# mravanelli/pytorch-kaldi

Hardware: AMD Instinct MI355X
Metric: train_frames_per_sec (higher is better)
Workload: dtype bf16

## Files before the change

include/pk_amd.h:

```cpp
#ifndef PK_AMD_H
#define PK_AMD_H

#include <stdint.h>

#ifdef __cplusplus
extern "C" {
#endif

#define PK_PREC_F32 0
#define PK_PREC_BF16 1

#define PK_ACT_LINEAR 0
#define PK_ACT_RELU 1
#define PK_ACT_TANH 2
#define PK_ACT_SIGMOID 3
#define PK_ACT_LEAKY_RELU 4
#define PK_ACT_ELU 5

#define PK_CELL_LIGRU 0
#define PK_CELL_RNN 1
#define PK_CELL_LSTM 2
#define PK_CELL_GRU 3
#define PK_CELL_MINGRU 4

#define PK_REC_STEPWISE 0
#define PK_REC_PERSISTENT 1

int pk_version(void);
const char* pk_last_error(void);
int pk_num_cu(void);

int pk_gemm(void* stream, int prec, int M, int N, int K, float alpha, const float* A, int64_t a_rs,
            int64_t a_cs, const float* B, int64_t b_rs, int64_t b_cs, float beta, float* C, int64_t ldc,
            const float* bias, int splitk, float* workspace);
void pk_gemm_f32_set_form(int form);

int pk_gemm_bf16_tile_m(int M);
int pk_gemm_bf16_auto_splitk(int M, int N, int K);
int pk_gemm_bf16_auto_splitk_cus(int M, int N, int K, int cus);
void pk_gemm_bf16_set_tile(int tile);
int pk_gemm_bf16(void* stream, int M, int N, int K, float alpha, const uint16_t* A, int64_t lda, int a_kc,
                 const uint16_t* B, int64_t ldb, int b_kc, float beta, float* C, int64_t ldc, const float* bias,
                 int splitk, float* workspace);
int64_t pk_gemm_bf16_stats_floats(int M, int N);
int pk_gemm_bf16_stats(void* stream, int M, int N, int K, float alpha, const uint16_t* A, int64_t lda, int a_kc,
                       const uint16_t* B, int64_t ldb, int b_kc, float* C, int64_t ldc, const float* bias, float* stats,
                       int* row_blocks);
int pk_cvt_bf16(void* stream, const float* src, int64_t ld_src, int64_t rows, int nseg, int seglen, int segpad,
                uint16_t* dst, int64_t ld_dst);

int64_t pk_bn_partial_floats(int64_t M, int64_t N);
int pk_bn_stats(void* stream, const float* x, int64_t ldx, int64_t M, int64_t N, float* partial, float* mean,
                float* var);
int pk_bn_stats_merge(void* stream, const float* partial, int rb, int64_t N, float* mean, float* var);
int pk_bn_finalize(void* stream, int64_t N, const float* mean, const float* var, const float* gamma,
                   const float* beta, float eps, float* scale, float* shift, float* running_mean,
                   float* running_var, float momentum, double count);
int pk_bn_finalize_gates(void* stream, int G, int H, const float* mean, const float* var, const float* gamma,
                         const float* beta, float eps, float* scale, float* shift, float* const* running_mean,
                         float* const* running_var, int64_t* const* num_batches, float momentum, double count);
int pk_bn_stats_merge_finalize_gates(void* stream, const float* partial, int rb, int G, int H, float* mean, float* var,
                                     const float* gamma, const float* beta, float eps, float* scale, float* shift,
                                     float* const* running_mean, float* const* running_var, int64_t* const* num_batches,
                                     float momentum, double count);
int pk_affine_act_fwd(void* stream, const float* x, int64_t ldx, int64_t M, int64_t N, const float* scale,
                      const float* shift, int act, const float* mask, float* y, int64_t ldy);
int pk_act_bwd(void* stream, const float* dy, const float* a, const float* mask, int act, int64_t n, float* g);
int pk_bn_bwd_reduce(void* stream, const float* g, const float* g2, int64_t ldg, const float* x, int64_t ldx,
                     int64_t M, int64_t N, const float* mean, const float* var, float eps, float* partial,
                     float* sum_g, float* sum_gx);
int pk_bn_bwd_apply(void* stream, const float* g, const float* g2, int64_t ldg, const float* x, int64_t ldx,
                    int64_t M, int64_t N, const float* mean, const float* var, float eps, const float* gamma,
                    const float* sum_g, const float* sum_gx, double count, float* dx, int64_t lddx);
int pk_bn_bwd_bf16(void* stream, const uint16_t* g0, const uint16_t* g1, int64_t g_pitch, int G, int H, const float* x,
                   int64_t ldx, int64_t M, const float* mean, const float* var, float eps, const float* gamma,
                   double count, float* partial, float* sum_g, float* sum_gx, uint16_t* out, int64_t out_pitch,
                   float* acc_beta, float* acc_gamma);
int pk_bn_act_bwd_small_covers(int64_t M, int64_t N);
int pk_bn_act_bwd_small(void* stream, const float* dy, const float* a, const float* mask, int act, const float* z,
                        const float* mean, const float* var, float eps, const float* gamma, int64_t M, int64_t N,
                        uint16_t* dzb, int64_t ldb, float* dz, float* sum_g, float* sum_gx, float* acc_beta,
                        float* acc_gamma, float* db, float* acc_bias);
int pk_colsum(void* stream, const float* g, const float* g2, int64_t ldg, int64_t M, int64_t N, float* partial,
              float* out);
int pk_add(void* stream, const float* a, const float* b, int64_t n, float* out);

int pk_mt19937_bernoulli(void* stream, uint32_t* state, int64_t n, float keep, float* out);

int pk_sinc_bank_fwd(void* stream, const float* low_hz, const float* band_hz, const float* n_, const float* window, int N, int K,
                     float sample_rate, float min_low, float min_band, float* filt, float* mx, int32_t* kstar);
int pk_sinc_bank_bwd(void* stream, const float* g, const float* low_hz, const float* band_hz, const float* n_, const float* window,
                     const float* mx, const int32_t* kstar, int N, int K, float sample_rate, float min_low, float min_band,
                     float* dlow, float* dband);
// ... 150 lines not shown
```

pytorch-kaldi_amd/_lib.py:

```python
import ctypes
import os
import re
import threading

HERE = os.path.dirname(os.path.abspath(__file__))
LIB_PATH = os.path.join(HERE, "lib", "libpk_amd.so")
HEADER = os.path.join(HERE, "..", "include", "pk_amd.h")

_lock = threading.Lock()
_lib = None

c_void_p, c_int, c_float, c_double, c_int64 = ctypes.c_void_p, ctypes.c_int, ctypes.c_float, ctypes.c_double, ctypes.c_int64
P = c_void_p

SIGNATURES = {
    "pk_version": (c_int, []),
    "pk_last_error": (ctypes.c_char_p, []),
    "pk_num_cu": (c_int, []),
    "pk_gemm": (c_int, [P, c_int, c_int, c_int, c_int, c_float, P, c_int64, c_int64, P, c_int64, c_int64, c_float, P,
                        c_int64, P, c_int, P]),
    "pk_gemm_f32_set_form": (None, [c_int]),
    "pk_gemm_bf16_tile_m": (c_int, [c_int]),
    "pk_gemm_bf16_auto_splitk": (c_int, [c_int, c_int, c_int]),
    "pk_gemm_bf16_set_tile": (None, [c_int]),
    "pk_gemm_bf16": (c_int, [P, c_int, c_int, c_int, c_float, P, c_int64, c_int, P, c_int64, c_int, c_float, P, c_int64, P,
                             c_int, P]),
    "pk_gemm_bf16_stats_floats": (c_int64, [c_int, c_int]),
    "pk_gemm_bf16_stats": (c_int, [P, c_int, c_int, c_int, c_float, P, c_int64, c_int, P, c_int64, c_int, P, c_int64, P, P, P]),
    "pk_bn_stats_merge": (c_int, [P, P, c_int, c_int64, P, P]),
    "pk_cvt_bf16": (c_int, [P, P, c_int64, c_int64, c_int, c_int, c_int, P, c_int64]),
    "pk_bn_partial_floats": (c_int64, [c_int64, c_int64]),
    "pk_bn_stats": (c_int, [P, P, c_int64, c_int64, c_int64, P, P, P]),
    "pk_bn_finalize": (c_int, [P, c_int64, P, P, P, P, c_float, P, P, P, P, c_float, c_double]),
    "pk_bn_finalize_gates": (c_int, [P, c_int, c_int, P, P, P, P, c_float, P, P, P, P, P, c_float, c_double]),
    "pk_bn_stats_merge_finalize_gates": (c_int, [P, P, c_int, c_int, c_int, P, P, P, P, c_float, P, P, P, P, P, c_float,
                                                 c_double]),
    "pk_affine_act_fwd": (c_int, [P, P, c_int64, c_int64, c_int64, P, P, c_int, P, P, c_int64]),
    "pk_act_bwd": (c_int, [P, P, P, P, c_int, c_int64, P]),
    "pk_bn_bwd_reduce": (c_int, [P, P, P, c_int64, P, c_int64, c_int64, c_int64, P, P, c_float, P, P, P]),
    "pk_bn_bwd_apply": (c_int, [P, P, P, c_int64, P, c_int64, c_int64, c_int64, P, P, c_float, P, P, P, c_double, P,
                                c_int64]),
    "pk_bn_bwd_bf16": (c_int, [P, P, P, c_int64, c_int, c_int, P, c_int64, c_int64, P, P, c_float, P, c_double, P, P, P, P,
                               c_int64, P, P]),
    "pk_colsum": (c_int, [P, P, P, c_int64, c_int64, c_int64, P, P]),
    "pk_add": (c_int, [P, P, P, c_int64, P]),
    "pk_mt19937_bernoulli": (c_int, [P, P, c_int64, c_float, P]),
    "pk_sinc_bank_fwd": (c_int, [P, P, P, P, P, c_int, c_int, c_float, c_float, c_float, P, P, P]),
    "pk_sinc_bank_bwd": (c_int, [P, P, P, P, P, P, P, P, c_int, c_int, c_float, c_float, c_float, P, P]),
    "pk_ln_last_act_drop_fwd": (c_int, [P, P, c_int64, c_int, c_int, P, P, c_float, c_int, P, P, P, P, P]),
    "pk_ln_last_act_drop_bwd": (c_int, [P, P, P, P, P, c_int64, c_int, c_int, P, P, P, c_float, c_int, P, P]),
    "pk_layernorm_fwd": (c_int, [P, P, c_int64, c_int64, P, P, c_float, P, P, P]),
    "pk_layernorm_bwd": (c_int, [P, P, P, c_int64, c_int64, P, P, P, c_float, P, P]),
    "pk_logsoftmax_fwd": (c_int, [P, P, c_int64, c_int64, P]),
    "pk_logsoftmax_bwd": (c_int, [P, P, P, c_int64, c_int64, P]),
    "pk_logsoftmax_bwd_ld": (c_int, [P, P, P, c_int64, c_int64, P, c_int64]),
    "pk_logsoftmax_fwd_ld": (c_int, [P, P, c_int64, c_int64, c_int64, P]),
    "pk_logsoftmax_fwd_ld_argmax": (c_int, [P, P, c_int64, c_int64, c_int64, P, P]),
    "pk_logsoftmax_bwd_bf16_partial_floats": (c_int64, [c_int64, c_int64]),
    "pk_logsoftmax_bwd_bf16": (c_int, [P, P, P, c_int64, c_int64, P, c_int64, P, P]),
    "pk_nll_err_partial_floats": (c_int64, [c_int64]),
    "pk_nll_err_fwd": (c_int, [P, P, P, c_int64, c_int64, c_int64, P, P, P, P]),
    "pk_nll_err_fwd_argmax": (c_int, [P, P, P, P, c_int64, c_int64, c_int64, P, P, P, P]),
    "pk_nll_logsoftmax_bwd_bf16": (c_int, [P, P, P, P, P, c_int64, c_int64, c_int64, P, c_int64, P, P]),
    "pk_logsoftmax_bwd_bf16_p": (c_int, [P, P, P, c_int64, c_int64, P, c_int64, c_int64, P, P]),
    "pk_nll_logsoftmax_bwd_bf16_p": (c_int, [P, P, P, P, P, c_int64, c_int64, c_int64, P, c_int64, c_int64, P, P]),
    "pk_rec_num_saved": (c_int, [c_int]),
    "pk_rec_num_gates": (c_int, [c_int]),
    "pk_conv1d_pool_dgrad": (c_int, [P, P, P, P, c_int, c_int, c_int, c_int, c_int, c_int, P, P]),
    "pk_conv_bf16_covers": (c_int, [c_int, c_int, c_int, c_int]),
    "pk_conv_bf16_work_floats": (c_int64, [c_int, c_int, c_int, c_int, c_int, c_int, c_int]),
    "pk_conv1d_pool_fwd_bf16": (c_int, [P, P, P, P, c_int, c_int, c_int, c_int, c_int, c_int, P, P, P]),
    "pk_conv1d_pool_bwd_bf16": (c_int, [P, P, P, P, P, c_int, c_int, c_int, c_int, c_int, c_int, P, P, P]),
    "pk_bn_act_bwd_small_covers": (c_int, [c_int64, c_int64]),
    "pk_bn_act_bwd_small": (c_int, [P, P, P, P, c_int, P, P, P, c_float, P, c_int64, c_int64, P, c_int64, P, P, P, P, P, P, P]),
    "pk_rec_work_floats": (c_int64, [c_int, c_int, c_int, c_int, c_int]),
    "pk_rec_ln_saved_floats": (c_int64, [c_int, c_int, c_int, c_int]),
    "pk_rec_ln_work_floats": (c_int64, [c_int, c_int, c_int, c_int]),
# ... 268 lines not shown
```

pytorch-kaldi_amd/csrc/pk_gemm_bf16.hip:

```cpp
#include <stdlib.h>

#include "pk_common.h"

namespace {

constexpr int TM = 128, TN = 128, TK = 64;
typedef short s4v __attribute__((ext_vector_type(4)));

struct BArgs {
    int M, N, K;
    float alpha, beta;
    const unsigned short* A;
    long lda;
    const unsigned short* B;
    long ldb;
    float* C;
    long ldc;
    const float* bias;
    float* ws;
    int k_per_split;
    int tiles_m, tiles_n;
    int items, per_xcd;
    const unsigned short* zeros;
    float* stats;
// ... 669 lines not shown
                bf16x8 a[2], b[2];
#pragma unroll
                for (int i = 0; i < 2; ++i) a[i] = frag_km32(cur + wm * 4096, i * 16, kk, lane);
#pragma unroll
                for (int j = 0; j < 2; ++j) b[j] = frag_km32(cur + 8192 + wn * 4096, j * 16, kk, lane);
#pragma unroll
                for (int i = 0; i < 2; ++i)
#pragma unroll
                    for (int j = 0; j < 2; ++j)
                        acc[i][j] = __builtin_amdgcn_mfma_f32_16x16x32_bf16(b[j], a[i], acc[i][j], 0, 0, 0);
            }
        }
        __syncthreads();
    }
    const bool vec_ok = (p.ldc & 3) == 0 && (((uintptr_t)p.C) & 15) == 0;
#pragma unroll
    for (int i = 0; i < 2; ++i) {
        const int row = m0 + wm * 32 + i * 16 + (lane & 15);
        if (row >= p.M) continue;
#pragma unroll
        for (int j = 0; j < 2; ++j) {
            const int col = n0 + wn * 32 + j * 16 + (lane >> 4) * 4;
            float* dst = p.C + (long)row * p.ldc + col;
            if (vec_ok && col + 3 < p.N) {
                f32x4 o;
#pragma unroll
                for (int r = 0; r < 4; ++r) o[r] = p.alpha * acc[i][j][r] + (p.bias ? p.bias[col + r] : 0.f);
                if (p.beta != 0.f) {
                    const f32x4 c = *reinterpret_cast<const f32x4*>(dst);
#pragma unroll
                    for (int r = 0; r < 4; ++r) o[r] += p.beta * c[r];
                }
                *reinterpret_cast<f32x4*>(dst) = o;
            } else {
#pragma unroll
                for (int r = 0; r < 4; ++r) {
                    if (col + r >= p.N) continue;
                    float o = p.alpha * acc[i][j][r] + (p.bias ? p.bias[col + r] : 0.f);
                    if (p.beta != 0.f) o += p.beta * dst[r];
                    dst[r] = o;
                }
            }
        }
    }
}

constexpr int PIECE = 16384;
template <int V>
struct BoolK {
    static constexpr int value = V;
};

typedef unsigned int u32x2v __attribute__((ext_vector_type(2)));
template <bool KC>
__device__ __forceinline__ bf16x8 frag8(const unsigned char* buf, int sub, int kk, int lane) {
    if (KC) {
        return frag<true>(buf, sub, kk, lane);
    } else {
        const int g = lane >> 4, i = lane & 15;
        const int col = sub + (i & 3) * 4;
        u32x2v h[2];
#pragma unroll
        for (int hh = 0; hh < 2; ++hh) {
            const int kr = kk * 32 + g * 8 + hh * 4 + (i >> 2);
            const int ps = (col >> 3) ^ swz_km(kr);
            const unsigned addr = (unsigned)(size_t)(const __attribute__((address_space(3))) unsigned char*)(buf + kr * 256 + ps * 16 + (col & 7) * 2);
            asm volatile("ds_read_b64_tr_b16 %0, %1" : "=v"(h[hh]) : "v"(addr) : "memory");
        }
        typedef unsigned int u32x4v __attribute__((ext_vector_type(4)));
        const u32x4v o = u32x4v{h[0][0], h[0][1], h[1][0], h[1][1]};
        return __builtin_bit_cast(bf16x8, o);
    }
}
template <bool ANY_ASM>
__device__ __forceinline__ void frag_wait() {
    if (ANY_ASM) {
        asm volatile("s_waitcnt lgkmcnt(0)" ::: "memory");
        __builtin_amdgcn_sched_barrier(0);
    }
}

template <bool KC>
struct PieceSrc {
    TileSrc<KC, 512> t;
    const unsigned short* base;
    long ld;
    int r0, rmax;
    __device__ __forceinline__ void init(const unsigned short* b, long l, int r0_, int rmax_, int k0, int tid) {
        base = b; ld = l; r0 = r0_; rmax = rmax_;
        t.init(b, l, r0_, rmax_, k0, tid);
    }
    template <bool CHECKED>
    __device__ __forceinline__ void issue(int k0, int kend, const unsigned short* zeros, unsigned char* slot, int tid, int wave) {
        if (!CHECKED || k0 + TK <= kend) {
            t.issue(slot, wave);
        } else {
            stage<KC, 512>(base, ld, r0, rmax, k0, kend, zeros, slot, tid, wave);
#pragma unroll
            for (int j = 0; j < 2; ++j) t.a[j] += t.step;
        }
    }
};

__device__ __forceinline__ void store_frag(const BArgs& p, const f32x4 v, int row, int col, int split, bool vec_ok) {
    if (row >= p.M || col >= p.N) return;
    float* dst = p.ws ? p.ws + ((long)split * p.M + row) * p.N + col : p.C + (long)row * p.ldc + col;
    if (vec_ok && col + 3 < p.N) {
        f32x4 o = v;
        if (p.ws == nullptr) {
#pragma unroll
            for (int r = 0; r < 4; ++r) o[r] = p.alpha * v[r] + (p.bias ? p.bias[col + r] : 0.f);
            if (p.beta != 0.f) {
                const f32x4 c = *reinterpret_cast<const f32x4*>(dst);
#pragma unroll
                for (int r = 0; r < 4; ++r) o[r] += p.beta * c[r];
            }
        }
        *reinterpret_cast<f32x4*>(dst) = o;
    } else {
#pragma unroll
        for (int r = 0; r < 4; ++r) {
            if (col + r >= p.N) continue;
            float o = v[r];
            if (p.ws == nullptr) {
                o = p.alpha * o + (p.bias ? p.bias[col + r] : 0.f);
                if (p.beta != 0.f) o += p.beta * dst[r];
            }
            dst[r] = o;
        }
    }
}

__device__ __forceinline__ void tile_colstats(const BArgs& p, const f32x4 (&acc)[2][2][4][2], int m0, int n0, int tm, int wm,
                                              int wn, int lane, float* sh) {
    const int nrows = (p.M - m0) < 256 ? (p.M - m0) : 256;
    __syncthreads();
    float part[2][2][4];
#pragma unroll
    for (int pass = 0; pass < 2; ++pass) {
        float mu[2][2][4];
        if (pass == 1) {
#pragma unroll
            for (int bh = 0; bh < 2; ++bh)
#pragma unroll
                for (int j = 0; j < 2; ++j)
#pragma unroll
                    for (int r = 0; r < 4; ++r) {
                        const int cl = bh * 128 + wn * 32 + j * 16 + (lane >> 4) * 4 + r;
                        mu[bh][j][r] = (sh[cl] + sh[256 + cl]) / (float)nrows;
                    }
        }
#pragma unroll
        for (int bh = 0; bh < 2; ++bh)
#pragma unroll
            for (int j = 0; j < 2; ++j)
#pragma unroll
                for (int r = 0; r < 4; ++r) {
                    float t = 0.f;
#pragma unroll
                    for (int ah = 0; ah < 2; ++ah)
#pragma unroll
                        for (int i = 0; i < 4; ++i) {
                            const bool in = ah * 128 + wm * 64 + i * 16 + (lane & 15) < nrows;
                            const float v = acc[ah][bh][i][j][r];
                            const float d = pass == 0 ? v : v - mu[bh][j][r];
                            t += in ? (pass == 0 ? d : d * d) : 0.f;
                        }
#pragma unroll
                    for (int off = 1; off < 16; off <<= 1) t += __shfl_xor(t, off);
                    part[bh][j][r] = t;
                }
        if ((lane & 15) == 0) {
#pragma unroll
            for (int bh = 0; bh < 2; ++bh)
#pragma unroll
                for (int j = 0; j < 2; ++j)
#pragma unroll
                    for (int r = 0; r < 4; ++r)
                        sh[pass * 512 + wm * 256 + bh * 128 + wn * 32 + j * 16 + (lane >> 4) * 4 + r] = part[bh][j][r];
        }
        __syncthreads();
    }
    const int c = threadIdx.x;
    if (c < 256 && n0 + c < p.N) {
        const float mean_v = (sh[c] + sh[256 + c]) / (float)nrows;
        const float m2_v = sh[512 + c] + sh[768 + c];
        float* o = p.stats + ((long)tm * p.N + n0 + c) * 3;
        o[0] = (float)nrows;
        o[1] = p.alpha * mean_v + (p.bias ? p.bias[n0 + c] : 0.f);
        o[2] = p.alpha * p.alpha * m2_v;
    }
}

#define PK_VMCNT(n) asm volatile("s_waitcnt vmcnt(" #n ")" ::: "memory")

template <bool A_KC, bool B_KC>
__global__ __launch_bounds__(512, 1) void gemm_bf16_256_kernel(BArgs p) {
    extern __shared__ __attribute__((aligned(1024))) unsigned char smem[];
    const int tid = threadIdx.x, lane = tid & 63, wave = tid >> 6;
    const int wm = wave >> 2, wn = wave & 3;
    const int item = (blockIdx.x & 7) * p.per_xcd + (blockIdx.x >> 3);
    if (item >= p.items) return;
    const int tn = item % p.tiles_n;
    const int tm = (item / p.tiles_n) % p.tiles_m;
    const int split = item / (p.tiles_n * p.tiles_m);
    const int m0 = tm * 256, n0 = tn * 256;
    const int kbeg = split * p.k_per_split;
    const int kend = min(p.K, kbeg + p.k_per_split);
    const int nk = (kend - kbeg + TK - 1) / TK;
    const bool a1_live = m0 + 128 < p.M, b1_live = n0 + 128 < p.N;

    f32x4 acc[2][2][4][2];
#pragma unroll
    for (int a = 0; a < 2; ++a)
#pragma unroll
        for (int b = 0; b < 2; ++b)
#pragma unroll
            for (int i = 0; i < 4; ++i)
#pragma unroll
                for (int j = 0; j < 2; ++j) acc[a][b][i][j] = f32x4{0.f, 0.f, 0.f, 0.f};

    PieceSrc<A_KC> sa0, sa1;
    PieceSrc<B_KC> sb0, sb1;
    sa0.init(p.A, p.lda, m0, p.M, kbeg, tid);
    sa1.init(p.A, p.lda, m0 + 128, p.M, kbeg, tid);
    sb0.init(p.B, p.ldb, n0, p.N, kbeg, tid);
    sb1.init(p.B, p.ldb, n0 + 128, p.N, kbeg, tid);
    auto slot = [&](int kt, int piece) { return smem + (((kt & 1) * 4 + piece) * PIECE); };
    auto issueA0 = [&](int kt, auto C) { sa0.template issue<decltype(C)::value != 0>(kbeg + kt * TK, kend, p.zeros, slot(kt, 0), tid, wave); };
    auto issueB0 = [&](int kt, auto C) { sb0.template issue<decltype(C)::value != 0>(kbeg + kt * TK, kend, p.zeros, slot(kt, 1), tid, wave); };
    auto issueB1 = [&](int kt, auto C) { sb1.template issue<decltype(C)::value != 0>(kbeg + kt * TK, kend, p.zeros, slot(kt, 2), tid, wave); };
    auto issueA1 = [&](int kt, auto C) { sa1.template issue<decltype(C)::value != 0>(kbeg + kt * TK, kend, p.zeros, slot(kt, 3), tid, wave); };

    issueA0(0, BoolK<1>()); issueB0(0, BoolK<1>()); issueB1(0, BoolK<1>()); issueA1(0, BoolK<1>());
    issueA0(1, BoolK<1>()); issueB0(1, BoolK<1>()); issueB1(1, BoolK<1>());
    PK_VMCNT(10);
    __builtin_amdgcn_s_barrier();
    if (wm == 1) __builtin_amdgcn_s_barrier();

    bf16x8 a[4][2], b[2][2][2];
#define PK_MFMA_BLOCK(AH, BH)                                                                                         \
    do {                                                                                                              \
// ... 9 lines not shown
        __builtin_amdgcn_sched_barrier(0);                 \
        __builtin_amdgcn_s_barrier();                      \
    } while (0)
    auto ktile = [&](int kt, auto FQC, auto CKC) {
        constexpr bool FQ = decltype(FQC)::value != 0;
        issueA1(kt + 1, CKC);
#pragma unroll
        for (int kk = 0; kk < 2; ++kk) {
#pragma unroll
            for (int j = 0; j < 2; ++j) b[0][j][kk] = frag8<B_KC>(slot(kt, 1), wn * 32 + j * 16, kk, lane);
#pragma unroll
            for (int i = 0; i < 4; ++i) a[i][kk] = frag8<A_KC>(slot(kt, 0), wm * 64 + i * 16, kk, lane);
        }
        PK_VMCNT(10);
        PK_END_L();
        PK_MFMA_BLOCK(0, 0);
        __builtin_amdgcn_s_barrier();
        issueA0(kt + 2, CKC);
#pragma unroll
        for (int kk = 0; kk < 2; ++kk)
#pragma unroll
            for (int j = 0; j < 2; ++j) b[1][j][kk] = frag8<B_KC>(slot(kt, 2), wn * 32 + j * 16, kk, lane);
        PK_VMCNT(10);
        PK_END_L();
        if (FQ || b1_live) PK_MFMA_BLOCK(0, 1);
        __builtin_amdgcn_s_barrier();
        issueB0(kt + 2, CKC);
#pragma unroll
        for (int kk = 0; kk < 2; ++kk)
#pragma unroll
            for (int i = 0; i < 4; ++i) a[i][kk] = frag8<A_KC>(slot(kt, 3), wm * 64 + i * 16, kk, lane);
        PK_END_L();
        if (FQ || (a1_live && b1_live)) PK_MFMA_BLOCK(1, 1);
        __builtin_amdgcn_s_barrier();
        issueB1(kt + 2, CKC);
        PK_VMCNT(10);
        __builtin_amdgcn_s_barrier();
        if (FQ || a1_live) PK_MFMA_BLOCK(1, 0);
        __builtin_amdgcn_s_barrier();
    };
    const int nk_full = (kend - kbeg) / TK;
    auto run = [&](auto FQC) {
        int kt = 0;
        for (; kt + 2 < nk_full; ++kt) ktile(kt, FQC, BoolK<0>());
        for (; kt < nk; ++kt) ktile(kt, FQC, BoolK<1>());
    };
    if (a1_live && b1_live) run(BoolK<1>());
    else run(BoolK<0>());
#undef PK_MFMA_BLOCK
#undef PK_END_L
    if (wm == 0) __builtin_amdgcn_s_barrier();
    PK_VMCNT(0);
    if constexpr (A_KC && B_KC) {
        if (p.stats != nullptr) tile_colstats(p, acc, m0, n0, tm, wm, wn, lane, reinterpret_cast<float*>(smem));
    }
    const bool vec_ok = (((uintptr_t)(p.ws ? p.ws : p.C) & 15) == 0) && (((p.ws ? (long)p.N : p.ldc) & 3) == 0);
    const bool interior = m0 + 256 <= p.M && n0 + 256 <= p.N;
    if (vec_ok && interior && (p.ws != nullptr || p.beta == 0.f)) {
        const bool direct = p.ws == nullptr;
        float* base = direct ? p.C : p.ws + (long)split * p.M * p.N;
        const long ld = direct ? p.ldc : (long)p.N;
        const float alpha = direct ? p.alpha : 1.f;
#pragma unroll
        for (int bh = 0; bh < 2; ++bh)
#pragma unroll
            for (int j = 0; j < 2; ++j) {
                const int col = n0 + bh * 128 + wn * 32 + j * 16 + (lane >> 4) * 4;
                f32x4 bv = f32x4{0.f, 0.f, 0.f, 0.f};
                if (direct && p.bias != nullptr) {
#pragma unroll
                    for (int r = 0; r < 4; ++r) bv[r] = p.bias[col + r];
                }
#pragma unroll
                for (int ah = 0; ah < 2; ++ah)
#pragma unroll
                    for (int i = 0; i < 4; ++i) {
                        const int row = m0 + ah * 128 + wm * 64 + i * 16 + (lane & 15);
                        const f32x4 v = acc[ah][bh][i][j];
                        f32x4 o;
#pragma unroll
                        for (int r = 0; r < 4; ++r) o[r] = alpha * v[r] + bv[r];
                        *reinterpret_cast<f32x4*>(base + (long)row * ld + col) = o;
                    }
            }
        return;
    }
#pragma unroll
    for (int ah = 0; ah < 2; ++ah)
#pragma unroll
        for (int bh = 0; bh < 2; ++bh)
#pragma unroll
            for (int i = 0; i < 4; ++i)
#pragma unroll
                for (int j = 0; j < 2; ++j)
                    store_frag(p, acc[ah][bh][i][j], m0 + ah * 128 + wm * 64 + i * 16 + (lane & 15),
                               n0 + bh * 128 + wn * 32 + j * 16 + (lane >> 4) * 4, split, vec_ok);
}

__global__ void splitk_reduce_bf_kernel(const float* __restrict__ ws, int splitk, int M, int N, float alpha, float beta,
                                        const float* __restrict__ bias, float* __restrict__ C, long ldc) {
    const long total = (long)M * N;
    if ((N & 3) == 0 && (ldc & 3) == 0 && (((uintptr_t)C | (uintptr_t)ws) & 15) == 0) {
        const long quads = total >> 2;
        for (long qd = blockIdx.x * (long)blockDim.x + threadIdx.x; qd < quads; qd += (long)gridDim.x * blockDim.x) {
            const long i = qd << 2;
            const int row = (int)(i / N), col = (int)(i - (long)row * N);
            f32x4 s = f32x4{0.f, 0.f, 0.f, 0.f};
            for (int k0 = 0; k0 < splitk; k0 += 8) {
                f32x4 t[8];
#pragma unroll
                for (int j = 0; j < 8; ++j) t[j] = *reinterpret_cast<const f32x4*>(ws + (long)(k0 + j < splitk ? k0 + j : splitk - 1) * total + i);
#pragma unroll
                for (int j = 0; j < 8; ++j)
#pragma unroll
                    for (int e = 0; e < 4; ++e) s[e] += (k0 + j < splitk) ? t[j][e] : 0.f;
            }
            float* c = C + (long)row * ldc + col;
            f32x4 o;
#pragma unroll
            for (int e = 0; e < 4; ++e) o[e] = alpha * s[e] + (bias ? bias[col + e] : 0.f);
            if (beta != 0.f) {
                const f32x4 cv = *reinterpret_cast<const f32x4*>(c);
#pragma unroll
                for (int e = 0; e < 4; ++e) o[e] += beta * cv[e];
            }
            *reinterpret_cast<f32x4*>(c) = o;
        }
        return;
    }
    for (long i = blockIdx.x * (long)blockDim.x + threadIdx.x; i < total; i += (long)gridDim.x * blockDim.x) {
        const int row = (int)(i / N), col = (int)(i % N);
        float s = 0.f;
        for (int k = 0; k < splitk; ++k) s += ws[(long)k * total + i];
        float o = alpha * s + (bias ? bias[col] : 0.f);
        float* c = C + (long)row * ldc + col;
        if (beta != 0.f) o += beta * (*c);
        *c = o;
    }
}

__global__ void cvt_bf16_kernel(const float* __restrict__ src, long lds, long rows, int nseg, int seglen, int segpad,
                                unsigned short* __restrict__ dst, long ldd) {
    const long chunks_per_row = ldd >> 3;
    const long total = rows * chunks_per_row;
    for (long i = blockIdx.x * (long)blockDim.x + threadIdx.x; i < total; i += (long)gridDim.x * blockDim.x) {
        const long r = i / chunks_per_row;
        const int c0 = (int)(i - r * chunks_per_row) * 8;
        const float* s = src + r * lds;
        unsigned pk[4];
#pragma unroll
        for (int e = 0; e < 4; ++e) {
            float v[2];
#pragma unroll
            for (int h = 0; h < 2; ++h) {
                const int c = c0 + 2 * e + h;
                const int sg = c / segpad, off = c - sg * segpad;
                v[h] = (sg < nseg && off < seglen) ? s[sg * seglen + off] : 0.f;
            }
            pk[e] = pk_pack_bf2(v[0], v[1]);
        }
        *reinterpret_cast<uint4*>(dst + r * ldd + c0) = make_uint4(pk[0], pk[1], pk[2], pk[3]);
    }
}

}

extern "C" int pk_cvt_bf16(void* stream, const float* src, int64_t ld_src, int64_t rows, int nseg, int seglen, int segpad,
                           uint16_t* dst, int64_t ld_dst) {
    if (rows <= 0) return 0;
    PK_REQUIRE(nseg >= 1 && seglen >= 1 && segpad >= seglen, "pk_cvt_bf16: bad segments");
    PK_REQUIRE((ld_dst % 8) == 0 && ld_dst >= (int64_t)nseg * segpad - (segpad - seglen) && ((uintptr_t)dst & 15) == 0,
               "pk_cvt_bf16: destination pitch must be a multiple of 8 elements and hold every segment");
    const long total = rows * (ld_dst >> 3);
    long blocks = (total + 255) / 256;
    if (blocks > 8192) blocks = 8192;
    hipLaunchKernelGGL(cvt_bf16_kernel, dim3((unsigned)blocks), dim3(256), 0, pk_stream(stream), src, (long)ld_src,
                       (long)rows, nseg, seglen, segpad, (unsigned short*)dst, (long)ld_dst);
    PK_LAUNCH_CHECK();
    return 0;
}

static int g_gemm_tile_forced = -1;
extern "C" void pk_gemm_bf16_set_tile(int tile) { g_gemm_tile_forced = (tile == 128 || tile == 256) ? tile : 0; }
static int gemm_tile_for(int M, int N, int a_kc, int b_kc, int K = 1 << 30) {
    int& forced = g_gemm_tile_forced;
    if (forced < 0) {
        const char* e = pk_experiment("gemm_tile");
        forced = (e && atoi(e) == 128) ? 128 : (e && atoi(e) == 256) ? 256 : 0;
    }
    if (forced) return forced;
    static int rows256 = -1;
    if (rows256 < 0) {
        const char* e = pk_experiment("gemm_tile_rows");
        rows256 = (e && atoi(e) == 0) ? 0 : 1;
    }
    if (rows256 && a_kc && M >= 16384 && N >= 1024) return 256;
    if (!a_kc && !b_kc && M >= 1024 && N >= 1024) {
        const long tiles256 = (long)((M + 255) / 256) * ((N + 255) / 256);
        if (K < 2048 && tiles256 < 64) return 128;
        return 256;
    }
    return 128;
}

extern "C" int pk_gemm_bf16_tile_m(int M) {
    (void)M;
    return TM;
}

extern "C" int pk_gemm_bf16_auto_splitk_cus(int M, int N, int K, int cus) {
    if (K < 2048 || M <= 0 || N <= 0) return 1;
    const int t = gemm_tile_for(M, N, 0, 0);
    const long tiles = (long)((M + t - 1) / t) * ((N + t - 1) / t);
    long ncu = pk_num_cu();
    if (cus > 0 && cus < ncu) ncu = cus;
    long s = (t == 256 ? ncu : 2 * ncu) / (tiles > 0 ? tiles : 1);
    if (s < 1) s = 1;
    if (s > 32) s = 32;
    const long kmax = K / 512 > 0 ? K / 512 : 1;
    if (s > kmax) s = kmax;
    return (int)s;
}
extern "C" int pk_gemm_bf16_auto_splitk(int M, int N, int K) { return pk_gemm_bf16_auto_splitk_cus(M, N, K, 0); }

static int gemm_bf16_impl(void* stream, int M, int N, int K, float alpha, const uint16_t* A, int64_t lda, int a_kc,
                          const uint16_t* B, int64_t ldb, int b_kc, float beta, float* C, int64_t ldc, const float* bias,
                          int splitk, float* workspace, float* stats) {
    if (M <= 0 || N <= 0) return 0;
    PK_REQUIRE(K >= 0, "pk_gemm_bf16: negative K");
    PK_REQUIRE((lda % 8) == 0 && (ldb % 8) == 0 && ((uintptr_t)A & 15) == 0 && ((uintptr_t)B & 15) == 0,
               "pk_gemm_bf16: operands need 16-byte aligned bases and pitches that are multiples of 8 elements");
    PK_REQUIRE(!a_kc || (K % 8) == 0 || lda >= ((K + 7) & ~7), "pk_gemm_bf16: A pitch shorter than K rounded up to 8");
    PK_REQUIRE(!b_kc || (K % 8) == 0 || ldb >= ((K + 7) & ~7), "pk_gemm_bf16: B pitch shorter than K rounded up to 8");
    PK_REQUIRE(a_kc || lda >= ((M + 7) & ~7), "pk_gemm_bf16: k-major A needs a pitch of at least M rounded up to 8");
    PK_REQUIRE(b_kc || ldb >= ((N + 7) & ~7), "pk_gemm_bf16: k-major B needs a pitch of at least N rounded up to 8");
    hipStream_t st = pk_stream(stream);
    BArgs p;
    p.M = M; p.N = N; p.K = K;
    p.alpha = alpha; p.beta = beta;
    p.A = A; p.lda = lda; p.B = B; p.ldb = ldb;
    p.C = C; p.ldc = ldc; p.bias = bias;
    p.stats = stats;
    const int tile = gemm_tile_for(M, N, a_kc, b_kc, K);
    PK_REQUIRE(stats == nullptr || (tile == 256 && a_kc && b_kc && splitk <= 1 && beta == 0.f), "pk_gemm_bf16_stats: internal: shape not covered");
    p.tiles_m = (M + tile - 1) / tile;
    p.tiles_n = (N + tile - 1) / tile;
    static void* zp = nullptr;
    if (zp == nullptr) PK_CHECK_HIP(hipGetSymbolAddress(&zp, HIP_SYMBOL(g_zero_page)));
    p.zeros = (const unsigned short*)zp;
    if (splitk < 1) splitk = 1;
    if (splitk > 1) {
        PK_REQUIRE(workspace != nullptr, "pk_gemm_bf16: split-K needs a workspace");
        int kps = (K + splitk - 1) / splitk;
        kps = ((kps + TK - 1) / TK) * TK;
        splitk = kps > 0 ? (K + kps - 1) / kps : 1;
        p.k_per_split = kps;
    }
    if (splitk <= 1) {
        splitk = 1;
        p.k_per_split = ((K + TK - 1) / TK) * TK;
        if (p.k_per_split == 0) p.k_per_split = TK;
    }
    p.ws = splitk > 1 ? workspace : nullptr;
    p.items = splitk * p.tiles_m * p.tiles_n;
    p.per_xcd = (p.items + 7) / 8;
    {
        static int skinny_on = -1;
        if (skinny_on < 0) {
            const char* e = pk_experiment("gemm_skinny");
            skinny_on = (e && e[0] == '0') ? 0 : 1;
        }
        if (skinny_on && !g_gemm_tile_forced && a_kc && M <= TM && splitk > 1 && p.k_per_split <= SK_TILES * TK && stats == nullptr) {
            static bool attr_done = false;
            if (!attr_done) {
                PK_CHECK_HIP(hipFuncSetAttribute((const void*)gemm_bf16sk_kernel<true>, hipFuncAttributeMaxDynamicSharedMemorySize, SK_TILES * SSTAGE));
                PK_CHECK_HIP(hipFuncSetAttribute((const void*)gemm_bf16sk_kernel<false>, hipFuncAttributeMaxDynamicSharedMemorySize, SK_TILES * SSTAGE));
                attr_done = true;
            }
            const dim3 sgrid((unsigned)((N + SN - 1) / SN), (unsigned)splitk);
            if (b_kc) hipLaunchKernelGGL((gemm_bf16sk_kernel<true>), sgrid, dim3(256), SK_TILES * SSTAGE, st, p);
            else hipLaunchKernelGGL((gemm_bf16sk_kernel<false>), sgrid, dim3(256), SK_TILES * SSTAGE, st, p);
            PK_LAUNCH_CHECK();
            const long total = (long)M * N;
            int blocks = (int)((total + 255) / 256);
            if (blocks > 2048) blocks = 2048;
            hipLaunchKernelGGL(splitk_reduce_bf_kernel, dim3(blocks), dim3(256), 0, st, workspace, splitk, M, N, alpha, beta,
                               bias, C, (long)ldc);
            PK_LAUNCH_CHECK();
            return 0;
        }
        if (skinny_on && !g_gemm_tile_forced && !a_kc && !b_kc && splitk == 1 && K <= 512 && stats == nullptr &&
            (long)((M + TM - 1) / TM) * ((N + TN - 1) / TN) <= 192 && M >= 64 && N >= 64) {
            const dim3 tgrid((unsigned)((N + 63) / 64), (unsigned)((M + 63) / 64));
            hipLaunchKernelGGL(gemm_bf16_t64_kernel, tgrid, dim3(256), T64_TILES * T64_STAGE, st, p);
            PK_LAUNCH_CHECK();
            return 0;
        }
        if (skinny_on && !g_gemm_tile_forced && a_kc && M <= TM && N >= 4 * SN && splitk == 1 && stats == nullptr) {
            BnActArgs q = {};
            const dim3 sgrid((unsigned)((N + SN - 1) / SN));
            if (b_kc) hipLaunchKernelGGL((gemm_bf16s_kernel<false, true>), sgrid, dim3(256), 2 * SSTAGE, st, p, q);
            else hipLaunchKernelGGL((gemm_bf16s_kernel<false, false>), sgrid, dim3(256), 2 * SSTAGE, st, p, q);
            PK_LAUNCH_CHECK();
            return 0;
        }
    }
    if (tile == 256) {
        static bool attr_done = false;
        if (!attr_done) {
            PK_CHECK_HIP(hipFuncSetAttribute((const void*)gemm_bf16_256_kernel<true, true>, hipFuncAttributeMaxDynamicSharedMemorySize, 8 * PIECE));
            PK_CHECK_HIP(hipFuncSetAttribute((const void*)gemm_bf16_256_kernel<true, false>, hipFuncAttributeMaxDynamicSharedMemorySize, 8 * PIECE));
            PK_CHECK_HIP(hipFuncSetAttribute((const void*)gemm_bf16_256_kernel<false, true>, hipFuncAttributeMaxDynamicSharedMemorySize, 8 * PIECE));
            PK_CHECK_HIP(hipFuncSetAttribute((const void*)gemm_bf16_256_kernel<false, false>, hipFuncAttributeMaxDynamicSharedMemorySize, 8 * PIECE));
            attr_done = true;
        }
        dim3 grid256((unsigned)(p.per_xcd * 8)), block512(512);
        const size_t lds256 = 8 * PIECE;
        if (a_kc && b_kc) hipLaunchKernelGGL((gemm_bf16_256_kernel<true, true>), grid256, block512, lds256, st, p);
        else if (a_kc && !b_kc) hipLaunchKernelGGL((gemm_bf16_256_kernel<true, false>), grid256, block512, lds256, st, p);
        else if (!a_kc && b_kc) hipLaunchKernelGGL((gemm_bf16_256_kernel<false, true>), grid256, block512, lds256, st, p);
        else hipLaunchKernelGGL((gemm_bf16_256_kernel<false, false>), grid256, block512, lds256, st, p);
        PK_LAUNCH_CHECK();
        if (splitk > 1) {
            const long total = (long)M * N;
            int blocks = (int)((total + 255) / 256);
            if (blocks > 2048) blocks = 2048;
            hipLaunchKernelGGL(splitk_reduce_bf_kernel, dim3(blocks), dim3(256), 0, st, workspace, splitk, M, N, alpha, beta,
                               bias, C, (long)ldc);
            PK_LAUNCH_CHECK();
        }
        return 0;
    }
    dim3 grid((unsigned)(p.per_xcd * 8)), block(256);
    static int forced = -1;
    if (forced < 0) {
        const char* e = pk_experiment("gemm_stages");
        forced = (e && e[0] == '1') ? 1 : (e && e[0] == '2') ? 2 : 0;
        PK_CHECK_HIP(hipFuncSetAttribute((const void*)gemm_bf16x_kernel<true, true, 2>, hipFuncAttributeMaxDynamicSharedMemorySize, 65536));
        PK_CHECK_HIP(hipFuncSetAttribute((const void*)gemm_bf16x_kernel<true, false, 2>, hipFuncAttributeMaxDynamicSharedMemorySize, 65536));
        PK_CHECK_HIP(hipFuncSetAttribute((const void*)gemm_bf16x_kernel<false, true, 2>, hipFuncAttributeMaxDynamicSharedMemorySize, 65536));
        PK_CHECK_HIP(hipFuncSetAttribute((const void*)gemm_bf16x_kernel<false, false, 2>, hipFuncAttributeMaxDynamicSharedMemorySize, 65536));
    }
    const int stages = forced ? forced : (a_kc ? 1 : 2);
    const size_t lds = stages == 2 ? 65536 : 32768;
#define PK_LAUNCH_BF(ST)                                                                                     \
    do {                                                                                                     \
        if (a_kc && b_kc) hipLaunchKernelGGL((gemm_bf16x_kernel<true, true, ST>), grid, block, lds, st, p);    \
        else if (a_kc && !b_kc) hipLaunchKernelGGL((gemm_bf16x_kernel<true, false, ST>), grid, block, lds, st, p); \
        else if (!a_kc && b_kc) hipLaunchKernelGGL((gemm_bf16x_kernel<false, true, ST>), grid, block, lds, st, p); \
        else hipLaunchKernelGGL((gemm_bf16x_kernel<false, false, ST>), grid, block, lds, st, p);              \
    } while (0)
    if (stages == 2) PK_LAUNCH_BF(2);
    else PK_LAUNCH_BF(1);
#undef PK_LAUNCH_BF
    PK_LAUNCH_CHECK();
    if (splitk > 1) {
        const long total = (long)M * N;
        int blocks = (int)((total + 255) / 256);
// ... 126 lines not shown
```

Baseline: 3.796 million.

## Add persistent 256-tile bf16 GEMM kernel with cross-tile prefetch pipelining

Adds a persistent bf16 GEMM kernel for 256x256 tiles. It launches one block per CU per XCD, and each block loops over several output tiles. The load pipeline keeps running across tile boundaries, so the next tile's A/B pieces are prefetched while the current tile's epilogue stores, and the bias vector is staged once in LDS. This is meant to remove per-tile launch, ramp-up and drain costs for large-M GEMMs (M>=16384, N>=1024, contiguous A). In exchange it adds complex vmcnt accounting that relies on a fixed count of epilogue stores, a larger LDS footprint, and the risk of uneven load across blocks.

```diff
diff --git a/include/pk_amd.h b/include/pk_amd.h
--- a/include/pk_amd.h
+++ b/include/pk_amd.h
@@ -39,6 +39,7 @@
 int pk_gemm_bf16_auto_splitk(int M, int N, int K);
 int pk_gemm_bf16_auto_splitk_cus(int M, int N, int K, int cus);
 void pk_gemm_bf16_set_tile(int tile);
+void pk_gemm_bf16_set_persist(int mode);
 int pk_gemm_bf16(void* stream, int M, int N, int K, float alpha, const uint16_t* A, int64_t lda, int a_kc,
                  const uint16_t* B, int64_t ldb, int b_kc, float beta, float* C, int64_t ldc, const float* bias,
                  int splitk, float* workspace);
diff --git a/pytorch-kaldi_amd/_lib.py b/pytorch-kaldi_amd/_lib.py
--- a/pytorch-kaldi_amd/_lib.py
+++ b/pytorch-kaldi_amd/_lib.py
@@ -23,6 +23,7 @@
     "pk_gemm_bf16_tile_m": (c_int, [c_int]),
     "pk_gemm_bf16_auto_splitk": (c_int, [c_int, c_int, c_int]),
     "pk_gemm_bf16_set_tile": (None, [c_int]),
+    "pk_gemm_bf16_set_persist": (None, [c_int]),
     "pk_gemm_bf16": (c_int, [P, c_int, c_int, c_int, c_float, P, c_int64, c_int, P, c_int64, c_int, c_float, P, c_int64, P,
                              c_int, P]),
     "pk_gemm_bf16_stats_floats": (c_int64, [c_int, c_int]),
diff --git a/pytorch-kaldi_amd/csrc/pk_gemm_bf16.hip b/pytorch-kaldi_amd/csrc/pk_gemm_bf16.hip
--- a/pytorch-kaldi_amd/csrc/pk_gemm_bf16.hip
+++ b/pytorch-kaldi_amd/csrc/pk_gemm_bf16.hip
@@ -745,6 +745,7 @@
 };
 
 typedef unsigned int u32x2v __attribute__((ext_vector_type(2)));
+typedef unsigned int u32x4v __attribute__((ext_vector_type(4)));
 template <bool KC>
 __device__ __forceinline__ bf16x8 frag8(const unsigned char* buf, int sub, int kk, int lane) {
     if (KC) {
@@ -760,7 +761,6 @@
             const unsigned addr = (unsigned)(size_t)(const __attribute__((address_space(3))) unsigned char*)(buf + kr * 256 + ps * 16 + (col & 7) * 2);
             asm volatile("ds_read_b64_tr_b16 %0, %1" : "=v"(h[hh]) : "v"(addr) : "memory");
         }
-        typedef unsigned int u32x4v __attribute__((ext_vector_type(4)));
         const u32x4v o = u32x4v{h[0][0], h[0][1], h[1][0], h[1][1]};
         return __builtin_bit_cast(bf16x8, o);
     }
@@ -795,14 +795,15 @@
     }
 };
 
-__device__ __forceinline__ void store_frag(const BArgs& p, const f32x4 v, int row, int col, int split, bool vec_ok) {
+__device__ __forceinline__ void store_frag(const BArgs& p, const f32x4 v, int row, int col, int split, bool vec_ok,
+                                           const float* bias) {
     if (row >= p.M || col >= p.N) return;
     float* dst = p.ws ? p.ws + ((long)split * p.M + row) * p.N + col : p.C + (long)row * p.ldc + col;
     if (vec_ok && col + 3 < p.N) {
         f32x4 o = v;
         if (p.ws == nullptr) {
 #pragma unroll
-            for (int r = 0; r < 4; ++r) o[r] = p.alpha * v[r] + (p.bias ? p.bias[col + r] : 0.f);
+            for (int r = 0; r < 4; ++r) o[r] = p.alpha * v[r] + (bias ? bias[col + r] : 0.f);
             if (p.beta != 0.f) {
                 const f32x4 c = *reinterpret_cast<const f32x4*>(dst);
 #pragma unroll
@@ -816,7 +817,7 @@
             if (col + r >= p.N) continue;
             float o = v[r];
             if (p.ws == nullptr) {
-                o = p.alpha * o + (p.bias ? p.bias[col + r] : 0.f);
+                o = p.alpha * o + (bias ? bias[col + r] : 0.f);
                 if (p.beta != 0.f) o += p.beta * dst[r];
             }
             dst[r] = o;
@@ -824,10 +825,11 @@
     }
 }
 
+template <bool LDS_BAR = false>
 __device__ __forceinline__ void tile_colstats(const BArgs& p, const f32x4 (&acc)[2][2][4][2], int m0, int n0, int tm, int wm,
-                                              int wn, int lane, float* sh) {
+                                              int wn, int lane, float* sh, const float* bias) {
     const int nrows = (p.M - m0) < 256 ? (p.M - m0) : 256;
-    __syncthreads();
+    if (LDS_BAR) asm volatile("s_waitcnt lgkmcnt(0)\n\ts_barrier" ::: "memory"); else __syncthreads();
     float part[2][2][4];
 #pragma unroll
     for (int pass = 0; pass < 2; ++pass) {
@@ -872,7 +874,7 @@
                     for (int r = 0; r < 4; ++r)
                         sh[pass * 512 + wm * 256 + bh * 128 + wn * 32 + j * 16 + (lane >> 4) * 4 + r] = part[bh][j][r];
         }
-        __syncthreads();
+        if (LDS_BAR) asm volatile("s_waitcnt lgkmcnt(0)\n\ts_barrier" ::: "memory"); else __syncthreads();
     }
     const int c = threadIdx.x;
     if (c < 256 && n0 + c < p.N) {
@@ -880,7 +882,7 @@
         const float m2_v = sh[512 + c] + sh[768 + c];
         float* o = p.stats + ((long)tm * p.N + n0 + c) * 3;
         o[0] = (float)nrows;
-        o[1] = p.alpha * mean_v + (p.bias ? p.bias[n0 + c] : 0.f);
+        o[1] = p.alpha * mean_v + (bias ? bias[n0 + c] : 0.f);
         o[2] = p.alpha * p.alpha * m2_v;
     }
 }
@@ -996,7 +998,7 @@
     if (wm == 0) __builtin_amdgcn_s_barrier();
     PK_VMCNT(0);
     if constexpr (A_KC && B_KC) {
-        if (p.stats != nullptr) tile_colstats(p, acc, m0, n0, tm, wm, wn, lane, reinterpret_cast<float*>(smem));
+        if (p.stats != nullptr) tile_colstats(p, acc, m0, n0, tm, wm, wn, lane, reinterpret_cast<float*>(smem), p.bias);
     }
     const bool vec_ok = (((uintptr_t)(p.ws ? p.ws : p.C) & 15) == 0) && (((p.ws ? (long)p.N : p.ldc) & 3) == 0);
     const bool interior = m0 + 256 <= p.M && n0 + 256 <= p.N;
@@ -1038,7 +1040,232 @@
 #pragma unroll
                 for (int j = 0; j < 2; ++j)
                     store_frag(p, acc[ah][bh][i][j], m0 + ah * 128 + wm * 64 + i * 16 + (lane & 15),
-                               n0 + bh * 128 + wn * 32 + j * 16 + (lane >> 4) * 4, split, vec_ok);
+                               n0 + bh * 128 + wn * 32 + j * 16 + (lane >> 4) * 4, split, vec_ok, p.bias);
+}
+
+constexpr int P_STORES = 32;
+constexpr int P_LDS_RING = 8 * PIECE, P_LDS_STATS = 4096;
+constexpr int P_LDS_MAX = 163840;
+constexpr int P_BIAS_MAX = (P_LDS_MAX - P_LDS_RING - P_LDS_STATS) / 4;
+
+template <bool B_KC>
+__global__ __launch_bounds__(512, 1) void gemm_bf16_256p_kernel(BArgs p) {
+    extern __shared__ __attribute__((aligned(1024))) unsigned char smem[];
+    float* const sh = reinterpret_cast<float*>(smem + P_LDS_RING);
+    float* const sbias = reinterpret_cast<float*>(smem + P_LDS_RING + P_LDS_STATS);
+    const int tid = threadIdx.x, lane = tid & 63, wave = tid >> 6;
+    const int wm = wave >> 2, wn = wave & 3;
+    const int xcd = blockIdx.x & 7, stride = gridDim.x >> 3, first = blockIdx.x >> 3;
+    const int chunk0 = xcd * p.per_xcd;
+    const int chunk = min(p.items - chunk0, p.per_xcd);
+    if (first >= chunk) return;
+    const int ntiles = (chunk - first + stride - 1) / stride;
+    const int kend = p.K;
+    const int nk = (kend + TK - 1) / TK, nk_full = kend / TK;
+    const bool stats = p.stats != nullptr;
+    const float* const bias = p.bias ? sbias : nullptr;
+
+    if (p.bias) {
+        for (int c = tid; c < p.N; c += 512) sbias[c] = p.bias[c];
+    }
+    __syncthreads();
+
+    auto tile_m0 = [&](int r) { return ((chunk0 + first + r * stride) / p.tiles_n) * 256; };
+    auto tile_n0 = [&](int r) { return ((chunk0 + first + r * stride) % p.tiles_n) * 256; };
+
+    PieceSrc<true> sa0, sa1;
+    PieceSrc<B_KC> sb0, sb1;
+    int ra0 = 0, ra1 = 0, rb0 = 0, rb1 = 0;
+    sa0.init(p.A, p.lda, tile_m0(0), p.M, 0, tid);
+    sa1.init(p.A, p.lda, tile_m0(0) + 128, p.M, 0, tid);
+    sb0.init(p.B, p.ldb, tile_n0(0), p.N, 0, tid);
+    sb1.init(p.B, p.ldb, tile_n0(0) + 128, p.N, 0, tid);
+    auto slot = [&](int g, int piece) { return smem + (((g & 1) * 4 + piece) * PIECE); };
+    auto issue_any = [&](auto& src, int& rcur, int piece, int g, bool is_a, int half) {
+        const int r = g / nk, kt = g - r * nk;
+        if (r >= ntiles) {
+            src.template issue<true>(kend, kend, p.zeros, slot(g, piece), tid, wave);
+            return;
+        }
+        if (r != rcur) {
+            rcur = r;
+            if (is_a) src.init(p.A, p.lda, tile_m0(r) + half * 128, p.M, kt * TK, tid);
+            else src.init(p.B, p.ldb, tile_n0(r) + half * 128, p.N, kt * TK, tid);
+        }
+        src.template issue<true>(kt * TK, kend, p.zeros, slot(g, piece), tid, wave);
+    };
+    auto issueA0 = [&](int g, auto C) { if (decltype(C)::value) issue_any(sa0, ra0, 0, g, true, 0); else sa0.template issue<false>(0, kend, p.zeros, slot(g, 0), tid, wave); };
+    auto issueB0 = [&](int g, auto C) { if (decltype(C)::value) issue_any(sb0, rb0, 1, g, false, 0); else sb0.template issue<false>(0, kend, p.zeros, slot(g, 1), tid, wave); };
+    auto issueB1 = [&](int g, auto C) { if (decltype(C)::value) issue_any(sb1, rb1, 2, g, false, 1); else sb1.template issue<false>(0, kend, p.zeros, slot(g, 2), tid, wave); };
+    auto issueA1 = [&](int g, auto C) { if (decltype(C)::value) issue_any(sa1, ra1, 3, g, true, 1); else sa1.template issue<false>(0, kend, p.zeros, slot(g, 3), tid, wave); };
+
+    issueA0(0, BoolK<1>()); issueB0(0, BoolK<1>()); issueB1(0, BoolK<1>()); issueA1(0, BoolK<1>());
+    issueA0(1, BoolK<1>()); issueB0(1, BoolK<1>()); issueB1(1, BoolK<1>());
+    PK_VMCNT(10);
+    __builtin_amdgcn_s_barrier();
+    if (wm == 1) __builtin_amdgcn_s_barrier();
+
+    f32x4 acc[2][2][4][2];
+    bf16x8 a[4][2], b[2][2][2];
+    bool a1_live = true, b1_live = true;
+    bool after_store = false;
+#define PK_MFMA_BLOCK(AH, BH)                                                                                         \
+    do {                                                                                                              \
+        __builtin_amdgcn_s_setprio(1);                                                                                \
+        _Pragma("unroll") for (int kk = 0; kk < 2; ++kk) _Pragma("unroll") for (int i = 0; i < 4; ++i)                   \
+            _Pragma("unroll") for (int j = 0; j < 2; ++j)                                                              \
+                acc[AH][BH][i][j] = __builtin_amdgcn_mfma_f32_16x16x32_bf16(b[BH][j][kk], a[i][kk], acc[AH][BH][i][j], 0, 0, 0); \
+        __builtin_amdgcn_s_setprio(0);                                                                                \
+    } while (0)
+#define PK_END_L()                                         \
+    do {                                                   \
+        asm volatile("s_waitcnt lgkmcnt(0)" ::: "memory"); \
+        __builtin_amdgcn_sched_barrier(0);                 \
+        __builtin_amdgcn_s_barrier();                      \
+    } while (0)
+#define PK_WAIT_PIECE(relax)                    \
+    do {                                        \
+        if (relax) PK_VMCNT(42);                \
+        else PK_VMCNT(10);                      \
+    } while (0)
+    static_assert(10 + P_STORES == 42 && 10 + P_STORES <= 63, "vmcnt(42) counts the straight-line epilogue's stores");
+    auto ktile = [&](int kt, int g, auto FQC, auto CKC) {
+        constexpr bool FQ = decltype(FQC)::value != 0;
+        const bool relax0 = after_store && kt == 0, relax1 = after_store && kt <= 1;
+        issueA1(g + 1, CKC);
+#pragma unroll
+        for (int kk = 0; kk < 2; ++kk) {
+#pragma unroll
+            for (int j = 0; j < 2; ++j) b[0][j][kk] = frag8<B_KC>(slot(g, 1), wn * 32 + j * 16, kk, lane);
+#pragma unroll
+            for (int i = 0; i < 4; ++i) a[i][kk] = frag8<true>(slot(g, 0), wm * 64 + i * 16, kk, lane);
+        }
+        PK_WAIT_PIECE(relax1);
+        PK_END_L();
+        PK_MFMA_BLOCK(0, 0);
+        __builtin_amdgcn_s_barrier();
+        issueA0(g + 2, CKC);
+#pragma unroll
+        for (int kk = 0; kk < 2; ++kk)
+#pragma unroll
+            for (int j = 0; j < 2; ++j) b[1][j][kk] = frag8<B_KC>(slot(g, 2), wn * 32 + j * 16, kk, lane);
+        PK_WAIT_PIECE(relax0);
+        PK_END_L();
+        if (FQ || b1_live) PK_MFMA_BLOCK(0, 1);
+        __builtin_amdgcn_s_barrier();
+        issueB0(g + 2, CKC);
+#pragma unroll
+        for (int kk = 0; kk < 2; ++kk)
+#pragma unroll
+            for (int i = 0; i < 4; ++i) a[i][kk] = frag8<true>(slot(g, 3), wm * 64 + i * 16, kk, lane);
+        PK_END_L();
+        if (FQ || (a1_live && b1_live)) PK_MFMA_BLOCK(1, 1);
+        __builtin_amdgcn_s_barrier();
+        issueB1(g + 2, CKC);
+        PK_WAIT_PIECE(relax0);
+        __builtin_amdgcn_s_barrier();
+        if (FQ || a1_live) PK_MFMA_BLOCK(1, 0);
+        __builtin_amdgcn_s_barrier();
+    };
+    for (int r = 0; r < ntiles; ++r) {
+        const int item = chunk0 + first + r * stride;
+        const int tm = item / p.tiles_n, tn = item - tm * p.tiles_n;
+        const int m0 = tm * 256, n0 = tn * 256;
+        const int g0 = r * nk;
+        const bool last = r + 1 == ntiles;
+        a1_live = m0 + 128 < p.M;
+        b1_live = n0 + 128 < p.N;
+#pragma unroll
+        for (int x = 0; x < 2; ++x)
+#pragma unroll
+            for (int y = 0; y < 2; ++y)
+#pragma unroll
+                for (int i = 0; i < 4; ++i)
+#pragma unroll
+                    for (int j = 0; j < 2; ++j) acc[x][y][i][j] = f32x4{0.f, 0.f, 0.f, 0.f};
+        auto run = [&](auto FQC) {
+            int kt = 0;
+            for (; kt + 2 < nk_full; ++kt) ktile(kt, g0 + kt, FQC, BoolK<0>());
+            for (; kt < nk; ++kt) ktile(kt, g0 + kt, FQC, BoolK<1>());
+        };
+        if (a1_live && b1_live) run(BoolK<1>());
+        else run(BoolK<0>());
+
+        if (wm == 0 && (stats || last)) __builtin_amdgcn_s_barrier();
+        if (stats) tile_colstats<true>(p, acc, m0, n0, tm, wm, wn, lane, sh, bias);
+        const bool vec_ok = ((uintptr_t)p.C & 15) == 0 && (p.ldc & 3) == 0;
+        const bool interior = m0 + 256 <= p.M && n0 + 256 <= p.N;
+        const long cbytes = (long)p.M * p.ldc * 4;
+        const bool edge_ok = vec_ok && p.beta == 0.f && !interior && cbytes <= 0x7fffffffL;
+        after_store = vec_ok && p.beta == 0.f && (interior || edge_ok);
+        if (after_store && interior) {
+#pragma unroll
+            for (int bh = 0; bh < 2; ++bh)
+#pragma unroll
+                for (int j = 0; j < 2; ++j) {
+                    const int col = n0 + bh * 128 + wn * 32 + j * 16 + (lane >> 4) * 4;
+                    f32x4 bv = f32x4{0.f, 0.f, 0.f, 0.f};
+                    if (bias != nullptr) bv = *reinterpret_cast<const f32x4*>(bias + col);
+#pragma unroll
+                    for (int ah = 0; ah < 2; ++ah)
+#pragma unroll
+                        for (int i = 0; i < 4; ++i) {
+                            const int row = m0 + ah * 128 + wm * 64 + i * 16 + (lane & 15);
+                            const f32x4 v = acc[ah][bh][i][j];
+                            f32x4 o;
+#pragma unroll
+                            for (int e = 0; e < 4; ++e) o[e] = p.alpha * v[e] + bv[e];
+                            *reinterpret_cast<f32x4*>(p.C + (long)row * p.ldc + col) = o;
+                        }
+                }
+        } else if (after_store) {
+            const __amdgpu_buffer_rsrc_t rc = __builtin_amdgcn_make_buffer_rsrc(p.C, 0, (int)cbytes, 0x00020000);
+            const int cq = (p.N - 1) & ~3;
+#pragma unroll
+            for (int bh = 0; bh < 2; ++bh)
+#pragma unroll
+                for (int j = 0; j < 2; ++j) {
+                    const int col = n0 + bh * 128 + wn * 32 + j * 16 + (lane >> 4) * 4;
+                    f32x4 bv = f32x4{0.f, 0.f, 0.f, 0.f};
+                    if (bias != nullptr) bv = *reinterpret_cast<const f32x4*>(bias + (col < cq ? col : cq));
+                    const bool full = col + 3 < p.N, part = col < p.N && !full;
+#pragma unroll
+                    for (int ah = 0; ah < 2; ++ah)
+#pragma unroll
+                        for (int i = 0; i < 4; ++i) {
+                            const int row = m0 + ah * 128 + wm * 64 + i * 16 + (lane & 15);
+                            const f32x4 v = acc[ah][bh][i][j];
+                            f32x4 o;
+#pragma unroll
+                            for (int e = 0; e < 4; ++e) o[e] = p.alpha * v[e] + bv[e];
+                            const bool in = row < p.M && full;
+                            const unsigned off = in ? (unsigned)(((long)row * p.ldc + col) * 4) : 0x80000000u;
+                            __builtin_amdgcn_raw_buffer_store_b128(__builtin_bit_cast(u32x4v, o), rc, (int)off, 0, 0);
+                            if (part && row < p.M) {
+#pragma unroll
+                                for (int e = 0; e < 3; ++e)
+                                    if (col + e < p.N) p.C[(long)row * p.ldc + col + e] = o[e];
+                            }
+                        }
+                }
+        } else {
+#pragma unroll
+            for (int ah = 0; ah < 2; ++ah)
+#pragma unroll
+                for (int bh = 0; bh < 2; ++bh)
+#pragma unroll
+                    for (int i = 0; i < 4; ++i)
+#pragma unroll
+                        for (int j = 0; j < 2; ++j)
+                            store_frag(p, acc[ah][bh][i][j], m0 + ah * 128 + wm * 64 + i * 16 + (lane & 15),
+                                       n0 + bh * 128 + wn * 32 + j * 16 + (lane >> 4) * 4, 0, vec_ok, bias);
+        }
+        if (wm == 1 && stats && !last) __builtin_amdgcn_s_barrier();
+    }
+#undef PK_MFMA_BLOCK
+#undef PK_END_L
+#undef PK_WAIT_PIECE
+    PK_VMCNT(0);
 }
 
 __global__ void splitk_reduce_bf_kernel(const float* __restrict__ ws, int splitk, int M, int N, float alpha, float beta,
@@ -1145,6 +1372,17 @@
         return 256;
     }
     return 128;
+}
+
+static int g_gemm_persist = -2;
+extern "C" void pk_gemm_bf16_set_persist(int mode) { g_gemm_persist = (mode == 0 || mode == 1) ? mode : -1; }
+static bool gemm_persist_for(int M, int N, int K, int a_kc, int splitk, const float* bias) {
+    if (g_gemm_persist == -2) {
+        const char* e = pk_experiment("gemm_persist");
+        g_gemm_persist = (e && e[0] == '0') ? 0 : (e && e[0] == '1') ? 1 : -1;
+    }
+    if (g_gemm_persist == 0 || !a_kc || splitk > 1 || K <= 0 || (bias != nullptr && N > P_BIAS_MAX)) return false;
+    return g_gemm_persist == 1 || (M >= 16384 && N >= 1024);
 }
 
 extern "C" int pk_gemm_bf16_tile_m(int M) {
@@ -1248,6 +1486,22 @@
             PK_LAUNCH_CHECK();
             return 0;
         }
+    }
+    if (tile == 256 && gemm_persist_for(M, N, K, a_kc, splitk, bias)) {
+        static bool attr_done = false;
+        if (!attr_done) {
+            PK_CHECK_HIP(hipFuncSetAttribute((const void*)gemm_bf16_256p_kernel<true>, hipFuncAttributeMaxDynamicSharedMemorySize, P_LDS_MAX));
+            PK_CHECK_HIP(hipFuncSetAttribute((const void*)gemm_bf16_256p_kernel<false>, hipFuncAttributeMaxDynamicSharedMemorySize, P_LDS_MAX));
+            attr_done = true;
+        }
+        int per = pk_num_cu() / 8;
+        if (per > p.per_xcd) per = p.per_xcd;
+        if (per < 1) per = 1;
+        const size_t lds = (size_t)P_LDS_RING + P_LDS_STATS + (bias ? (size_t)((N + 3) & ~3) * 4 : 0);
+        if (b_kc) hipLaunchKernelGGL((gemm_bf16_256p_kernel<true>), dim3((unsigned)(8 * per)), dim3(512), lds, st, p);
+        else hipLaunchKernelGGL((gemm_bf16_256p_kernel<false>), dim3((unsigned)(8 * per)), dim3(512), lds, st, p);
+        PK_LAUNCH_CHECK();
+        return 0;
     }
     if (tile == 256) {
         static bool attr_done = false;
```

New measurement: 3.844 million (median of 6 runs). 1.01x the previous value.
